# razayunus/ManhattanSLAM

Hardware: AMD Instinct MI355X
Metric: RGB-D frames/sec at 640x480 (ORB+surfel front end) (higher is better)
Workload: dtype u8/i32 (ORB)/f32+f64 (surfel)

## Files before the change

manhattanslam_amd/csrc/msl_sf.h:

```cpp
#pragma once

#include "msl_common.h"

#include <hip/hip_ext.h>

namespace msl {
namespace sf {

constexpr int SP = 8;
constexpr int NCHUNK = 10;
constexpr double MAX_ANGLE_COS = 0.1, HUBER_RANGE = 0.4, MIN_TOLERATE_DIFF = 0.1;
constexpr unsigned T_INF = 0xFFFFFFFFu;
constexpr int PROP_ROUNDS = 6;
constexpr unsigned short IDX_NONE = 0xFFFF, IDX_PLANE = 0xFFFE;
constexpr int LIST_D = 256;
constexpr int SCAN_ITEMS = 1024;
#ifndef MSL_SUB_ITEMS
#define MSL_SUB_ITEMS 128
#endif
constexpr int SUB_ITEMS = MSL_SUB_ITEMS;
constexpr int DEFER_WIN = 32;
#ifndef MSL_FUSEREC_PLANES
#define MSL_FUSEREC_PLANES 0
#endif
__host__ __device__ inline size_t fuserec_index(int nseeds, unsigned seed, int word) {
#if MSL_FUSEREC_PLANES
    return (size_t)word * (size_t)nseeds + seed;
#else
    (void)nseeds; return 3 * (size_t)seed + (size_t)word;
#endif
}

struct alignas(16) HotPk { float px, py, pz; unsigned tl; };
struct HotRec { float px, py, pz; int updateTimes, lastUpdate; };
constexpr unsigned HOT_WIDE = 0x80000000u, HOT_HOLE = 0xFFFFFFFFu;
__host__ __device__ inline bool tl_fits(int ut, int lu) { return (unsigned)ut < 2048u && ((unsigned)lu + (1u << 19)) < (1u << 20); }
__host__ __device__ inline unsigned tl_pack(int ut, int lu) { return ((unsigned)ut << 20) | ((unsigned)lu & 0xFFFFFu); }
__host__ __device__ inline int tl_ut(unsigned tl) { return (int)(tl >> 20); }
__host__ __device__ inline int tl_lu(unsigned tl) { return (int)(tl << 12) >> 12; }
struct alignas(32) ColdRec { float nx, ny, nz, size, color, weight; unsigned rgbf; unsigned _spare; };
constexpr unsigned COLD_WIDE = 1u << 24;
struct MapSoA {
    HotPk *hot;
    ColdRec *cold;
    int *rgbWide;
    int *utlWide;
    long long *wideFlag;
};
__host__ __device__ inline bool rgb_fits(int r, int g, int b) { return ((unsigned)r | (unsigned)g | (unsigned)b) < 256u; }
__host__ __device__ inline unsigned rgb_pack(int r, int g, int b) { return (unsigned)r | ((unsigned)g << 8) | ((unsigned)b << 16); }

template <typename T> using gptr = const T __attribute__((address_space(1))) *;
struct FrameDev {
    const uint8_t *gray; const float *depth; const int32_t *member;
    float pose[16], invPose[16];
    int ref, _pad;
#ifdef __HIPCC__
    __device__ __forceinline__ gptr<uint8_t> grayG() const { return (gptr<uint8_t>)gray; }
    __device__ __forceinline__ gptr<float> depthG() const { return (gptr<float>)depth; }
    __device__ __forceinline__ gptr<int32_t> memberG() const { return (gptr<int32_t>)member; }
#endif
};

struct alignas(32) AssignRec {
    float x, y, meanIntensity;
    unsigned stable;
    double invDepth;
    unsigned long long _pad;
};

struct FuseAux {
    MapSoA map;
    unsigned long long cap;
// ... 179 lines not shown
```

manhattanslam_amd/csrc/msl_sf_map.hip:

```cpp

#include "msl_sf.h"

using namespace msl;
using namespace msl::sf;

namespace {

__device__ __forceinline__ unsigned ld_agent(const unsigned *p) { return __hip_atomic_load(p, __ATOMIC_RELAXED, __HIP_MEMORY_SCOPE_AGENT); }
__device__ __forceinline__ void st_agent(unsigned *p, unsigned v) { __hip_atomic_store(p, v, __ATOMIC_RELAXED, __HIP_MEMORY_SCOPE_AGENT); }
__device__ __forceinline__ unsigned long long ld_agent64(const unsigned long long *p) { return __hip_atomic_load(p, __ATOMIC_RELAXED, __HIP_MEMORY_SCOPE_AGENT); }
__device__ __forceinline__ void st_agent64(unsigned long long *p, unsigned long long v) { __hip_atomic_store(p, v, __ATOMIC_RELAXED, __HIP_MEMORY_SCOPE_AGENT); }

__device__ __forceinline__ void set_wide_flag_ptr(long long *flag, unsigned long long bit) { atomicOr(reinterpret_cast<unsigned long long *>(flag), bit); }
__device__ __forceinline__ void set_wide_flag(const MapSoA &M, unsigned long long bit) { set_wide_flag_ptr(M.wideFlag, bit); }
__device__ __forceinline__ void tl_unpack(const MapSoA &M, long long i, unsigned tl, int &ut, int &lu) {
    ut = tl_ut(tl); lu = tl_lu(tl);
    if (tl & 0x80000000u) {
        if (tl == HOT_WIDE) { ut = M.utlWide[2 * i]; lu = M.utlWide[2 * i + 1]; }
        else { ut = 0; lu = 0; }
    }
}
__device__ __forceinline__ HotRec hot_load(const MapSoA &M, long long i) {
    const HotPk p = M.hot[i];
    HotRec h; h.px = p.px; h.py = p.py; h.pz = p.pz;
// ... 39 lines not shown
    ColdRec c; c.nx = e.nx; c.ny = e.ny; c.nz = e.nz; c.size = e.size; c.color = e.color; c.weight = e.weight; c._spare = 0;
    if (rgb_fits(e.r, e.g, e.b)) c.rgbf = rgb_pack(e.r, e.g, e.b);
    else { c.rgbf = COLD_WIDE; set_wide_flag(M, 1ull); M.rgbWide[3 * i] = e.r; M.rgbWide[3 * i + 1] = e.g; M.rgbWide[3 * i + 2] = e.b; }
    hot_store(M, i, h); cold_store(M.cold + i, c);
}
__device__ __forceinline__ void load_surfel(const MapSoA &M, long long i, const HotRec &h, msl_surfel &e) {
    const ColdRec c = cold_load(M.cold + i);
    e.px = h.px; e.py = h.py; e.pz = h.pz; e.nx = c.nx; e.ny = c.ny; e.nz = c.nz; e.size = c.size; e.color = c.color;
    if (c.rgbf & COLD_WIDE) { e.r = M.rgbWide[3 * i]; e.g = M.rgbWide[3 * i + 1]; e.b = M.rgbWide[3 * i + 2]; }
    else { e.r = (int)(c.rgbf & 255u); e.g = (int)((c.rgbf >> 8) & 255u); e.b = (int)((c.rgbf >> 16) & 255u); }
    e.weight = c.weight; e.updateTimes = h.updateTimes; e.lastUpdate = h.lastUpdate;
}
__device__ __forceinline__ void move_surfel(const MapSoA &M, long long dst, long long src) {
    const ColdRec c = cold_load(M.cold + src);
    const HotPk p = M.hot[src];
    M.hot[dst] = p; cold_store(M.cold + dst, c);
    if (p.tl == HOT_WIDE) { M.utlWide[2 * dst] = M.utlWide[2 * src]; M.utlWide[2 * dst + 1] = M.utlWide[2 * src + 1]; }
    if (c.rgbf & COLD_WIDE) { M.rgbWide[3 * dst] = M.rgbWide[3 * src]; M.rgbWide[3 * dst + 1] = M.rgbWide[3 * src + 1]; M.rgbWide[3 * dst + 2] = M.rgbWide[3 * src + 2]; }
}

__device__ __forceinline__ bool last_workgroup(unsigned *ticket, unsigned *s_flag) {
    asm volatile("s_waitcnt vmcnt(0)" ::: "memory");
    __syncthreads();
    if (threadIdx.x == 0) {
        const unsigned t = atomicAdd(ticket, 1u);
        *s_flag = (t == gridDim.x - 1) ? 1u : 0u;
        if (*s_flag) __hip_atomic_store(ticket, 0u, __ATOMIC_RELAXED, __HIP_MEMORY_SCOPE_AGENT);
    }
    __syncthreads();
    return *s_flag != 0;
}

__device__ __forceinline__ int round_half_up_pixel(float u) {
    const float c = fminf(fmaxf(u, -4.0f), 1.0e6f);
    const float f = floorf(c);
    return (int)f + ((c - f) >= 0.5f ? 1 : 0);
}
__device__ __forceinline__ unsigned lane_rank(unsigned long long m) {
    return __builtin_amdgcn_mbcnt_hi((unsigned)(m >> 32), __builtin_amdgcn_mbcnt_lo((unsigned)m, 0u));
}

typedef unsigned u32x4 __attribute__((ext_vector_type(4)));
__device__ __forceinline__ void st16(void *p, u32x4 v) { *reinterpret_cast<u32x4 *>(p) = v; }

struct FuseFrame {
    float inv[12];
    int ref;
    const FrameDev *frame;
};
struct FuseArgs {
    int W, H, nseeds, kf;
    int prevSlot;
    int rowScale;
    float fx, fy, cx, cy, fuseFar, fuseNear;
    const uint2 *tex; const float4 *fuseRec; uint8_t *fused;
    HotPk *hot; ColdRec *cold;
    long long *ctr;
    unsigned *blockSums, *blockUpd;
    unsigned *sbKeys;
    const unsigned *deal;
    unsigned *delOut;
    unsigned *delCount;
    DeferCtl *dc;
};
__host__ inline FuseArgs fuse_args(const SfDev &P, int slot, bool deferred, bool dealt = false) {
    FuseArgs A;
    A.W = P.W; A.H = P.H; A.nseeds = P.nseeds; A.kf = P.kf; A.prevSlot = P.prevSlotAbs; A.rowScale = (254 << 16) / P.H;
    A.sbKeys = P.sbKeys; A.deal = dealt ? P.deal : nullptr;
    A.fx = P.fx; A.fy = P.fy; A.cx = P.cx; A.cy = P.cy; A.fuseFar = P.fuseFar; A.fuseNear = P.fuseNear;
    A.tex = P.tex + (size_t)slot * P.pxStride; A.fuseRec = P.fuseRec + (size_t)slot * P.nseeds * 3; A.fused = P.fused + (size_t)slot * P.flagStride;
    A.hot = P.map.hot; A.cold = P.map.cold; A.ctr = P.ctr;
    A.dc = P.dc;
    A.blockSums = P.blockSums; A.blockUpd = P.blockUpd + (size_t)(deferred ? P.kf : 0) * (P.cap / SUB_ITEMS + 8200);
    A.delOut = deferred ? P.delList : P.delU;
    A.delCount = deferred ? &P.dc->delCnt[P.kf < DEFER_WIN ? P.kf : 0] : P.delUCount;
    return A;
}
__host__ inline FuseFrame fuse_frame(const FrameDev &F, const FrameDev *dev) {
    FuseFrame f;
    for (int c = 0; c < 4; c++) for (int r = 0; r < 3; r++) f.inv[3 * c + r] = F.invPose[4 * c + r];
    f.ref = F.ref; f.frame = dev;
    return f;
}
__device__ __forceinline__ void mul4r(const float *m, float v0, float v1, float v2, float v3, float out[3]) {
#pragma unroll
    for (int r = 0; r < 3; r++) out[r] = ((m[r] * v0 + m[3 + r] * v1) + m[6 + r] * v2) + m[9 + r] * v3;
}
__device__ __forceinline__ void mul3r(const float *m, float v0, float v1, float v2, float out[3]) {
#pragma unroll
    for (int r = 0; r < 3; r++) out[r] = (m[r] * v0 + m[3 + r] * v1) + m[6 + r] * v2;
}

__device__ __forceinline__ unsigned spawn_word(unsigned fw) { return ~(fw | (fw >> 1)) & 0x01010101u; }
__device__ __forceinline__ unsigned spawn_count(const FuseArgs &P, unsigned lane, unsigned &excl) {
    const DeferCtl *dc = P.dc;
    const int fs = dc->flagStride;
    const uint8_t *fusedP = dc->fused + (size_t)P.prevSlot * fs;
    const int per = fs >> 6, nch = per >> 4;
    unsigned cnt = 0;
    const uint4 *fq = reinterpret_cast<const uint4 *>(fusedP + (size_t)lane * per);
    for (int c = 0; c < nch; c += 5) {
        uint4 b[5];
#pragma unroll
        for (int q = 0; q < 5; q++) b[q] = fq[min(c + q, nch - 1)];
#pragma unroll
        for (int q = 0; q < 5; q++)
            if (c + q < nch) cnt += (unsigned)(__popc(spawn_word(b[q].x)) + __popc(spawn_word(b[q].y)) + __popc(spawn_word(b[q].z)) + __popc(spawn_word(b[q].w)));
    }
    const unsigned incl = wave_incl_scan(cnt);
    excl = incl - cnt;
    return (unsigned)__builtin_amdgcn_readlane((int)incl, 63);
}
__device__ __forceinline__ void emit_records(const FuseArgs &P, long long E0, long long c0, int nj, unsigned lane, unsigned K, unsigned excl) {
    const DeferCtl *dc = P.dc;
    const int fs = dc->flagStride;
    const uint8_t *fusedP = dc->fused + (size_t)P.prevSlot * fs;
    const int per = fs >> 6, nch = per >> 4;
    const msl_surfel *cand = dc->cand + (size_t)P.prevSlot * P.nseeds;
#pragma unroll 1
    for (int j = 0; j < nj; j++) {
        const long long i = c0 + 64 * j + lane, kS = i - E0;
        const bool on = kS >= 0 && kS < (long long)K;
        const unsigned k = on ? (unsigned)kS : 0u;
        unsigned lo = 0, hi = 63, eLo = 0;
#pragma unroll
        for (int s = 0; s < 6; s++) {
            const unsigned mid = (lo + hi + 1) >> 1;
            const unsigned e = (unsigned)__builtin_amdgcn_ds_bpermute((int)(mid * 4u), (int)excl);
            if (e <= k) { lo = mid; eLo = e; } else hi = mid - 1;
        }
        unsigned r = k - eLo;
        int seed = -1;
        const uint4 *of = reinterpret_cast<const uint4 *>(fusedP + (size_t)lo * per);
        for (int c = 0; c < nch; c++) {
            const uint4 b = of[c];
            const unsigned w[4] = {spawn_word(b.x), spawn_word(b.y), spawn_word(b.z), spawn_word(b.w)};
#pragma unroll
            for (int q = 0; q < 4; q++) {
                const unsigned pc = (unsigned)__popc(w[q]);
                if (seed < 0) {
                    if (r < pc) {
                        unsigned m = w[q];
                        for (unsigned t = 0; t < r; t++) m &= m - 1;
                        seed = (int)lo * per + 16 * c + 4 * q + (__builtin_ctz(m) >> 3);
                    } else r -= pc;
                }
            }
        }
        if (on && seed >= 0) {
            if ((unsigned long long)i < dc->aux.cap) store_surfel(dc->aux.map, i, cand[seed]);
            else { long long code = 20; asm volatile("" : "+v"(code)); P.ctr[5] = code; }
        }
    }
    asm volatile("s_waitcnt vmcnt(0)" ::: "memory");
}

template <bool DEFER, bool spawnWave>
__device__ __forceinline__ void fuse_body(const FuseArgs &P, const FuseFrame &F, int nSubHint, unsigned waveIdx, int G) {
    constexpr int KPL = SUB_ITEMS / 64;
    constexpr long long WSPAN = 64 * KPL;
    struct { HotPk *hot; ColdRec *cold; } M = {P.hot, P.cold};
    const FuseAux *aux = &P.dc->aux;
    const unsigned lane0 = threadIdx.x;
    const uint2 *tex = P.tex;
    const float4 *fuseRec = P.fuseRec;
    uint8_t *fused = P.fused;
    const int ref = F.ref;
    const float cameraF = (float)(((double)fabsf(P.fx) + (double)fabsf(P.fy)) / 2.0);
    const float halfF = 0.5f * cameraF;
    const bool pending = DEFER && P.kf > 0;
    long long E0v = 0;
    if (pending) E0v = P.dc->ext[P.kf - 1];
    long long E0 = 0;
    if (DEFER && spawnWave) E0 = ((long long)__builtin_amdgcn_readfirstlane((int)(E0v >> 32)) << 32) | (unsigned)__builtin_amdgcn_readfirstlane((int)E0v);
    if (spawnWave && !pending) return;
    if (DEFER && !pending && waveIdx == 0 && lane0 == 0) P.dc->ext[0] = P.ctr[0];
    if (DEFER && !spawnWave && waveIdx == 0 && lane0 == 0) P.dc->logBase[P.kf] = P.kf > 0 ? P.dc->logBase[P.kf - 1] + P.dc->delCnt[P.kf - 1] : 0u;
    unsigned spK = 0;
    if (DEFER && spawnWave) {
        unsigned excl;
        spK = spawn_count(P, lane0, excl);
        if (lane0 == 0) P.dc->ext[P.kf] = E0 + (long long)spK;
        if (spK == 0) return;
    }
#ifndef MSL_FUSE_CHUNK
#define MSL_FUSE_CHUNK 16
#endif
    constexpr unsigned FUSE_CHUNK = MSL_FUSE_CHUNK;
    long long sb0;
    if (!spawnWave && P.deal != nullptr) {
        const unsigned gs = (unsigned)G >> 3;
        const unsigned *dp = P.deal + ((waveIdx & 7u) * gs + (waveIdx >> 3));
        unsigned dv;
        asm volatile("s_load_dword %0, %1, 0x0\n\ts_waitcnt lgkmcnt(0)" : "=s"(dv) : "s"(dp) : "memory");
        sb0 = (long long)dv;
    } else {
        long long lin = waveIdx;
        constexpr unsigned T = 8u * FUSE_CHUNK;
        const unsigned full = ((unsigned)G / T) * T;
        if (waveIdx < full) { const unsigned grp = waveIdx / T, r = waveIdx % T; lin = (long long)grp * T + (r & 7u) * FUSE_CHUNK + (r >> 3); }
        sb0 = (long long)G - 1 - lin;
    }
    for (long long it = 0;; it++) {
        unsigned lane = lane0;
        asm volatile("" : "+v"(lane));
#define REC_LOCAL(k) (64u * (unsigned)(k) + lane)
        const long long sb = sb0 + it * G;
        long long c0, n = 0, cntIdx;
        if (DEFER && spawnWave) {
            c0 = E0 + it * WSPAN;
            n = E0 + (long long)spK;
            if (c0 >= n) return;
            unsigned excl;
            (void)spawn_count(P, lane, excl);
            emit_records(P, E0, c0, KPL, lane, spK, excl);
            cntIdx = E0 / SUB_ITEMS + 1 + it;
        } else {
            c0 = sb * WSPAN; cntIdx = sb;
            if (pending) {
                if (it > 0) {
                    E0 = ((long long)__builtin_amdgcn_readfirstlane((int)(E0v >> 32)) << 32) | (unsigned)__builtin_amdgcn_readfirstlane((int)E0v);
                    if (c0 >= E0) return;
                }
            } else if (sb >= nSubHint && c0 >= __hip_atomic_load(&P.ctr[0], __ATOMIC_RELAXED, __HIP_MEMORY_SCOPE_AGENT)) return;
        }
        HotPk hq[KPL];
#pragma unroll
        for (int k = 0; k < KPL; k++) hq[k] = M.hot[c0 + REC_LOCAL(k)];
        if (!pending) n = P.ctr[0];
        else if (!spawnWave) {
            E0 = ((long long)__builtin_amdgcn_readfirstlane((int)(E0v >> 32)) << 32) | (unsigned)__builtin_amdgcn_readfirstlane((int)E0v);
            if (c0 >= E0) return;
            n = E0;
        }
        unsigned stp = 0;
        unsigned keyAcc = 0;
        float pzv[KPL];
        unsigned offT[KPL];
        unsigned anyTl = 0;
#pragma unroll
        for (int k = 0; k < KPL; k++) anyTl |= hq[k].tl;
        const bool anyHi = __builtin_expect(__ballot(anyTl >> 31) != 0ull, 0);
#pragma unroll
        for (int k = 0; k < KPL; k++) {
            const long long i = c0 + REC_LOCAL(k);
            const float x = hq[k].px, y = hq[k].py, z = hq[k].pz;
            const unsigned tl = hq[k].tl;
            int ut = tl_ut(tl), lu = tl_lu(tl);
            bool hole = false;
            if (anyHi) {
                if (tl == HOT_WIDE) { const int *w = aux->map.utlWide; ut = w[2 * i]; lu = w[2 * i + 1]; }
                else if (tl & 0x80000000u) hole = true;
            }
            float pc[3];
            mul4r(F.inv, x, y, z, 1.0f, pc);
            const bool inRange = !(pc[2] < P.fuseNear || pc[2] > P.fuseFar);
            const bool live = i < n && !hole, stale = ref - lu > 5 && ut < 5;
            int st = 0;
            if (live) st = stale ? (ut != 0 ? 1 : 2) : (ut == 0 ? 2 : 0);
            const bool cand = live && !stale && ut != 0 && inRange;
            unsigned off = 0;
            {
                const float zq = inRange ? pc[2] : 1.0f;
                const float projectU = pc[0] * P.fx / zq + P.cx, projectV = pc[1] * P.fy / zq + P.cy;
                const int pUInt = round_half_up_pixel(projectU), pVInt = round_half_up_pixel(projectV);
                const bool inImage = !(pUInt < 1 || pUInt > P.W - 2 || pVInt < 1 || pVInt > P.H - 2);
                if (cand && inImage) { st = 3; keyAcc += (((unsigned)pVInt * (unsigned)P.rowScale) >> 16) | 0x10000u; }
                off = st == 3 ? (unsigned)(pVInt * P.W + pUInt) : 0u;
            }
            stp |= (unsigned)st << (2 * k); pzv[k] = pc[2];
            offT[k] = off;
        }
        uint2 tx[KPL];
        {
#pragma unroll
            for (int k = 0; k < KPL; k++) tx[k] = tex[offT[k]];
            if constexpr (KPL == 4) asm volatile("" ::"v"(tx[0].x), "v"(tx[1].x), "v"(tx[2].x), "v"(tx[3].x), "v"(tx[0].y), "v"(tx[1].y), "v"(tx[2].y), "v"(tx[3].y));
            else asm volatile("" ::"v"(tx[0].x), "v"(tx[KPL - 1].x), "v"(tx[0].y), "v"(tx[KPL - 1].y));
        }
        if (!(DEFER && spawnWave)) {
            const unsigned ks = (unsigned)__builtin_amdgcn_readlane((int)wave_incl_scan(keyAcc), 63);
            const unsigned kc = ks >> 16;
            const unsigned key = kc ? min((unsigned)((float)(ks & 0xFFFFu) * __builtin_amdgcn_rcpf((float)kc)), 254u) : 255u;
            if (lane == 0) P.sbKeys[cntIdx] = key;
        }
        unsigned fl = 0;
        unsigned cntDel = 0;
#pragma unroll
        for (int k = 0; k < KPL; k++) {
            const unsigned st = (stp >> (2 * k)) & 3u;
            const bool occluded = st == 3u && (double)pzv[k] < (double)__uint_as_float(tx[k].x) - 1.0;
            const bool del = st == 1u || st == 2u || occluded;
            if (DEFER) { if (del) M.hot[c0 + REC_LOCAL(k)].tl = HOT_HOLE; }
            else if (st == 1u || occluded) {
                if (__builtin_expect(hq[k].tl == HOT_WIDE, 0)) aux->map.utlWide[2 * (c0 + REC_LOCAL(k))] = 0;
                else M.hot[c0 + REC_LOCAL(k)].tl = hq[k].tl & 0xFFFFFu;
            }
            fl |= del ? (1u << k) : 0u;
            fl |= (st == 3u && !occluded) ? (16u << k) : 0u;
            cntDel += (unsigned)__popcll(__ballot(del));
        }
        auto list_base = [&](unsigned c) -> unsigned {
            unsigned base = 0, prior = 0;
            if (DEFER && P.kf > 0) prior = P.dc->logBase[P.kf - 1] + P.dc->delCnt[P.kf - 1];
            if (lane == 0) base = atomicAdd(P.delCount, c);
            return (unsigned)__builtin_amdgcn_readfirstlane((int)base) + prior;
        };
        auto hand_over = [&](bool d, unsigned long long m, unsigned base, long long i) {
            if (d) {
                const unsigned j = base + lane_rank(m);
                if (DEFER || j < (unsigned)LIST_D) P.delOut[j] = (unsigned)i;
            }
        };
        if (cntDel) {
            unsigned base = list_base(cntDel);
#pragma unroll
            for (int k = 0; k < KPL; k++) {
                const bool d = (fl >> k) & 1u;
                const unsigned long long m = __ballot(d);
                hand_over(d, m, base, c0 + REC_LOCAL(k)); base += (unsigned)__popcll(m);
            }
        }
        unsigned rcv[KPL], bk[KPL];
        unsigned total = 0;
#pragma unroll
        for (int k = 0; k < KPL; k++) {
            const bool sv = (fl >> (4 + k)) & 1u;
            const unsigned long long m = __ballot(sv);
            const unsigned c = (unsigned)__popcll(m), rs = lane_rank(m);
// ... 44 lines not shown
                        const float newWeight = f1.w;
                        const float sumWeight = oldWeight + newWeight;
                        const float fusedPx = (h.px * oldWeight + newWeight * f1.x) / sumWeight;
                        const float fusedPy = (h.py * oldWeight + newWeight * f1.y) / sumWeight;
                        const float fusedPz = (h.pz * oldWeight + newWeight * f1.z) / sumWeight;
                        float fusedNx = nc[0] * oldWeight + newWeight * f0.x;
                        float fusedNy = nc[1] * oldWeight + newWeight * f0.y;
                        float fusedNz = nc[2] * oldWeight + newWeight * f0.z;
                        const float newNormLength = sqrtf(fusedNx * fusedNx + fusedNy * fusedNy + fusedNz * fusedNz);
                        fusedNx = fusedNx / newNormLength; fusedNy = fusedNy / newNormLength; fusedNz = fusedNz / newNormLength;
                        float newNormW[3];
                        newNormW[0] = (r00 * fusedNx + r01 * fusedNy) + r02 * fusedNz;
                        newNormW[1] = (r10 * fusedNx + r11 * fusedNy) + r12 * fusedNz;
                        newNormW[2] = (r20 * fusedNx + r21 * fusedNy) + r22 * fusedNz;
                        int ut = (int)(h.tl >> 20);
                        if (__builtin_expect(h.tl == HOT_WIDE, 0)) ut = aux->map.utlWide[2 * i];
                        unsigned tlNew = tl_pack(ut + 1, ref);
                        if (__builtin_expect(!tl_fits(ut + 1, ref), 0)) {
                            int *w = aux->map.utlWide;
                            w[2 * i] = ut + 1; w[2 * i + 1] = ref;
                            asm volatile("" ::: "memory");
                            set_wide_flag_ptr(aux->map.wideFlag, 2ull);
                            tlNew = HOT_WIDE;
                        }
                        c.rgbf = __float_as_uint(f2.z);
                        c.nx = newNormW[0]; c.ny = newNormW[1]; c.nz = newNormW[2];
                        c.weight = sumWeight;
                        c.color = f2.y;
                        const float newSize = f2.x;
                        if (newSize < c.size) c.size = newSize;
                        u32x4 hv = {__float_as_uint(fusedPx), __float_as_uint(fusedPy), __float_as_uint(fusedPz), tlNew};
                        u32x4 c0v = {__float_as_uint(c.nx), __float_as_uint(c.ny), __float_as_uint(c.nz), __float_as_uint(c.size)};
                        u32x4 c1v = {__float_as_uint(c.color), __float_as_uint(c.weight), c.rgbf, 0u};
                        st16(M.hot + i, hv);
                        st16(M.cold + i, c0v);
                        st16(reinterpret_cast<u32x4 *>(M.cold + i) + 1, c1v);
                        fused[sp] = 1;
                        upd = true;
                    }
                }
            }
            nupd += (unsigned)__popcll(__ballot(upd));
            const unsigned long long mb = __ballot(delB);
            if (mb) {
                const unsigned cb = (unsigned)__popcll(mb);
                hand_over(delB, mb, list_base(cb), i);
                cntDelB += cb;
            }
        }
        if (lane == 0) {
            if (!DEFER) P.blockSums[cntIdx] = cntDel + cntDelB;
            P.blockUpd[cntIdx] = nupd;
        }
        if (!(DEFER && spawnWave) && (sb + G) * WSPAN >= n) return;
    }
#undef REC_LOCAL
}

template <bool DEFER>
__global__ __launch_bounds__(64) __attribute__((amdgpu_waves_per_eu(6, 8))) void k_fuse(FuseArgs P, FuseFrame F, int nSubHint) {
    __builtin_amdgcn_s_setprio(3);
    if (DEFER) {
        if (blockIdx.x == 0) fuse_body<DEFER, true>(P, F, nSubHint, 0u, (int)gridDim.x - 1);
        else fuse_body<DEFER, false>(P, F, nSubHint, blockIdx.x - 1u, (int)gridDim.x - 1);
    } else {
        fuse_body<false, false>(P, F, nSubHint, blockIdx.x, (int)gridDim.x);
    }
}

template <int NT>
__device__ __forceinline__ void deal_subblocks(const unsigned *keys, int G, unsigned *deal, unsigned *s_hist, unsigned *s_off, unsigned *s_wave, unsigned *s_aux) {
    static_assert(NT == 256, "one histogram bin per thread");
    const unsigned t = threadIdx.x;
    constexpr int CH = 32 * NT;
    auto load_pack = [&](int base, unsigned (&kp)[8]) {
        uint4 v[8];
#pragma unroll
        for (int q = 0; q < 8; q++) v[q] = *reinterpret_cast<const uint4 *>(keys + base + 32 * (int)t + 4 * q);
#pragma unroll
        for (int q = 0; q < 8; q++) kp[q] = min(v[q].x, 255u) | (min(v[q].y, 255u) << 8) | (min(v[q].z, 255u) << 16) | (min(v[q].w, 255u) << 24);
    };
    auto next_word = [&](unsigned (&kp)[8]) -> unsigned {
        const unsigned w = kp[0];
#pragma unroll
        for (int q = 0; q < 7; q++) kp[q] = kp[q + 1];
        kp[7] = w;
        return w;
    };
    auto count_chunk = [&](int base, unsigned (&kp)[8], bool hist) -> unsigned {
        unsigned fc = 0;
#pragma unroll 1
        for (int d = 0; d < 8; d++) {
            const unsigned w = next_word(kp);
#pragma unroll
            for (int b = 0; b < 4; b++) {
                const unsigned key = (w >> (8 * b)) & 255u;
                const bool in = base + 32 * (int)t + 4 * d + b < G;
                if (hist && in && key != 255u) atomicAdd(&s_hist[key], 1u);
                fc += in && key == 255u ? 1u : 0u;
            }
        }
        return fc;
    };
    unsigned k0[8];
    load_pack(0, k0);
    s_hist[t] = 0;
    __syncthreads();
    const unsigned fc0 = count_chunk(0, k0, true);
    for (int base = CH; base < G; base += CH) { unsigned kc[8]; load_pack(base, kc); (void)count_chunk(base, kc, true); }
    __syncthreads();
    unsigned NI, fTot0, ex, fb0;
    block_excl_scan_pair(t < 255u ? s_hist[t] : 0u, fc0, s_wave, &NI, &fTot0, ex, fb0);
    const unsigned gs = (unsigned)G >> 3;
    auto inS = [&](unsigned x) { return (x * NI + 7u) >> 3; };
    auto outS = [&](unsigned x) { return x * gs - inS(x); };
    {
        unsigned x0 = 0;
#pragma unroll
        for (unsigned y = 1; y < 8; y++) x0 += ex >= inS(y) ? 1u : 0u;
// ... 700 lines not shown
    load_surfel(M, i, h, e);
    dst[i] = e;
}
__global__ void k_set_ctr(long long *ctr, long long n, unsigned *delUCount, int wide) {
    if (threadIdx.x == 0) {
        delUCount[0] = 0;
        ctr[0] = n; ctr[1] = 0; ctr[2] = 0; ctr[3] = 0; ctr[4] = n; ctr[6] = n; ctr[7] = 0;
        if (wide >= 0) ctr[13] = wide;
    }
}

__global__ __launch_bounds__(64) void k_collect_changed(SfDev P, int ref, long long n, unsigned *count, unsigned *idxOut, msl_surfel *recOut, unsigned capOut) {
    const long long sb = blockIdx.x;
    if (!(P.blockSums[sb] | P.blockUpd[sb])) return;
    const unsigned lane = threadIdx.x;
    for (int k = 0; k < SUB_ITEMS / 64; k++) {
        const long long i = sb * SUB_ITEMS + k * 64 + lane;
        HotRec h; h.px = h.py = h.pz = 0; h.updateTimes = 1; h.lastUpdate = ref - 1;
        if (i < n) h = hot_load(P.map, i);
        const bool ch = i < n && (h.updateTimes == 0 || h.lastUpdate == ref);
        const unsigned long long m = __ballot(ch);
        if (!m) continue;
        unsigned base = 0;
        if (lane == 0) base = atomicAdd(count, (unsigned)__popcll(m));
        base = __builtin_amdgcn_readfirstlane(base);
        if (ch) {
            const unsigned j = base + lane_rank(m);
            if (j < capOut) { msl_surfel e; load_surfel(P.map, i, h, e); recOut[j] = e; idxOut[j] = (unsigned)i; }
        }
    }
}

__global__ void k_empty(int grid_dummy) { (void)grid_dummy; }

}

namespace msl {
namespace sf {

void map_launch_deal(hipStream_t st, const SfDev &P) { hipLaunchKernelGGL(k_deal, dim3(1), dim3(256), 0, st, P.sbKeys, P.dealG, P.deal); }
int map_debug_deal(const uint32_t *keys_host, int G, uint32_t *deal_host) {
    if (!keys_host || !deal_host || G < 8 || (G & 7)) return MSL_ERR_INVALID;
    const size_t pad = (size_t)G + 8192;
    DevBuf keys, deal;
    MSL_HIP_TRY(grow_all(0, {{keys, sizeof(unsigned) * pad}, {deal, sizeof(unsigned) * (G + 64)}}));
    unsigned *dk = (unsigned *)keys.p, *dd = (unsigned *)deal.p;
    MSL_HIP_TRY(hipMemset(dk, 0xFF, sizeof(unsigned) * pad)); MSL_HIP_TRY(hipMemset(dd, 0xFF, sizeof(unsigned) * G));
    MSL_HIP_TRY(hipMemcpy(dk, keys_host, sizeof(unsigned) * G, hipMemcpyHostToDevice));
    hipLaunchKernelGGL(k_deal, dim3(1), dim3(256), 0, 0, dk, G, dd);
    MSL_HIP_TRY(hipGetLastError());
    MSL_HIP_TRY(hipMemcpy(deal_host, dd, sizeof(unsigned) * G, hipMemcpyDeviceToHost));
    return MSL_OK;
}
void map_launch_fuse(KernelProfiler &prof, hipStream_t st, const SfDev &P, int slot, const FrameDev &F, int nSubGrid, int nSubHint, bool deferred, bool dealt) {
    const FuseArgs A = fuse_args(P, slot, deferred, dealt);
    const FuseFrame FF = fuse_frame(F, P.frames + slot);
    if (deferred) MSL_SF_LAUNCH(prof, SK_FUSE, st, k_fuse<true>, dim3((unsigned)nSubGrid + 1u), dim3(64), A, FF, nSubHint);
    else MSL_SF_LAUNCH(prof, SK_FUSE, st, k_fuse<false>, dim3((unsigned)nSubGrid), dim3(64), A, FF, nSubHint);
}
void map_launch_compact(KernelProfiler &prof, hipStream_t st, const SfDev &P, int slot, bool resident) {
    const CompactArgs A = compact_args(P, slot);
    const int per = (((P.nseeds + 255) / 256) + 3) & ~3;
    const bool aligned4 = (P.nseeds & 3) == 0 && ((reinterpret_cast<size_t>(A.candOk) | reinterpret_cast<size_t>(A.fused)) & 3) == 0;
    const dim3 grid(resident ? 128 : 1);
    if (per <= 32 && aligned4) MSL_SF_LAUNCH(prof, SK_COMPACT, st, k_compact<8>, grid, dim3(256), A, resident ? 0 : 1);
    else if (per <= 96 && aligned4) MSL_SF_LAUNCH(prof, SK_COMPACT, st, k_compact<24>, grid, dim3(256), A, resident ? 0 : 1);
    else MSL_SF_LAUNCH(prof, SK_COMPACT, st, k_compact<0>, grid, dim3(256), A, resident ? 0 : 1);
}
void map_launch_replay(KernelProfiler &prof, hipStream_t st, const SfDev &P, int F, unsigned blkStride) {
    const unsigned nFront = (unsigned)((P.nseeds + SUB_ITEMS - 1) / SUB_ITEMS) + 1u;
    hipLaunchKernelGGL(k_defer_tail, dim3((unsigned)F + nFront), dim3(64), 0, st, P, fuse_args(P, 0, true), F, blkStride);
    MSL_SF_LAUNCH(prof, SK_COMPACT, st, k_replay, dim3(1), dim3(64), P, F);
    hipLaunchKernelGGL(k_gather, dim3(128), dim3(256), 0, st, P);
    hipLaunchKernelGGL(k_scatter, dim3(128), dim3(256), 0, st, P);
}
void map_launch_empty_pair(KernelProfiler &prof, hipStream_t st) {
    hipEvent_t ea, eb;
    if (prof.kernel_pair(SK_NEW, &ea, &eb)) hipExtLaunchKernelGGL(k_empty, dim3(1), dim3(64), 0, st, ea, eb, 0, 0);
}
void map_launch_set_ctr(hipStream_t st, const SfDev &P, long long n, int wide) { hipLaunchKernelGGL(k_set_ctr, dim3(1), dim3(64), 0, st, P.ctr, n, P.delUCount, wide); }
void map_launch_add_ctr(hipStream_t st, const SfDev &P, long long add) { hipLaunchKernelGGL(k_add_ctr, dim3(1), dim3(64), 0, st, P.ctr, add); }
void map_launch_aos_to_soa(KernelProfiler &prof, hipStream_t st, const SfDev &P, const msl_surfel *src, long long n, bool atEnd) {
    if (atEnd) hipLaunchKernelGGL(k_aos_to_soa_at, dim3((unsigned)((n + 255) / 256)), dim3(256), 0, st, P.map, src, n, P.ctr);
    else MSL_SF_LAUNCH(prof, SK_CONVERT, st, k_aos_to_soa, dim3((unsigned)((n + 255) / 256)), dim3(256), P.map, src, n);
}
void map_launch_soa_to_aos(KernelProfiler &prof, hipStream_t st, const SfDev &P, msl_surfel *dst, long long n) {
    MSL_SF_LAUNCH(prof, SK_CONVERT, st, k_soa_to_aos, dim3((unsigned)((n + 255) / 256)), dim3(256), P.map, dst, n);
}
void map_launch_select_count(hipStream_t st, const SfDev &P, int mode, int arg) {
    hipLaunchKernelGGL(k_select_count, dim3(512), dim3(256), 0, st, P, mode, arg);
    hipLaunchKernelGGL(k_select_scan, dim3(1), dim3(1024), 0, st, P);
}
void map_launch_select_write(hipStream_t st, const SfDev &P, int mode, int arg, msl_surfel *out, int markDeleted) {
    hipLaunchKernelGGL(k_select_write, dim3(512), dim3(256), 0, st, P, mode, arg, out, markDeleted);
}
void map_launch_collect_changed(hipStream_t st, const SfDev &P, int ref, long long n, unsigned *count, unsigned *idxOut, msl_surfel *recOut, unsigned capOut) {
    const unsigned nblk = (unsigned)((n + SUB_ITEMS - 1) / SUB_ITEMS);
    hipLaunchKernelGGL(k_collect_changed, dim3(nblk), dim3(64), 0, st, P, ref, n, count, idxOut, recOut, capOut);
}
void map_launch_empty(hipStream_t st, int grid, hipEvent_t a, hipEvent_t b) { hipExtLaunchKernelGGL(k_empty, dim3((unsigned)grid), dim3(64), 0, st, a, b, 0, grid); }

}
}
```

manhattanslam_amd/csrc/msl_surfel.hip:

```cpp

#include "msl_sf.h"

#include <algorithm>
#include <cmath>
#include <cstdlib>
#include <fstream>
#include <memory>
#include <new>
#include <vector>

using namespace msl;
using namespace msl::sf;

namespace {
const char *kSfNames[MSL_SF_NKERNELS] = {"kb_seed_init", "kb_assign", "kb_prop", "kb_commit_px", "kb_update_seeds", "kb_commit_seeds",
                                         "kb_seed_plane", "k_fuse", "k_empty", "k_compact", "k_convert", "copy"};
}

struct msl_sf {
    int device = 0;
    SfDev dev{};
    int maxBatch = 1;
    hipStream_t preStream = nullptr, mapStream = nullptr; bool ownStreams = true;
    size_t blkStride = 0;
    unsigned long long kfClassic = 0, kfDeferred = 0;
    int dealG = 0;
    hipStream_t copyStream = nullptr;
    hipEvent_t evH2D[2] = {nullptr, nullptr};
    hipEvent_t evPre[2] = {nullptr, nullptr}, evMap[2] = {nullptr, nullptr}, evCopy[2] = {nullptr, nullptr};
    bool evMapValid[2] = {false, false}, evCopyValid[2] = {false, false}, evPreValid[2] = {false, false};
    unsigned long long batchNo = 0;
    int stagedSet = -1; size_t stagedGs = 0;
    int lastSlot = 0;
    struct Slots {
        DevBuf frames, seeds, seedsTmp, cand, candOk, fused, tex, fuseRec, index, amap, tmin, arec, pxInv, wl, wlCount, chunkAbort, changed;
        PinBuf hFrames;
        DevBuf gray, depth, member;
        size_t grayCap = 0, depthCap = 0, memberCap = 0;
        DevBuf depth16; size_t depth16Cap = 0;
    } slot;
    DevBuf d_ctr; PinBuf h_ctr;
    DevBuf d_tickets, d_delU, d_dc, d_projTab;
    bool propLds = false;
    bool classicNext = true;
    DevBuf d_new;
    struct MapBufs { DevBuf store, blockSums, blockUpd, delList, srcOf, rp; } map;
    size_t liveBound = 0;
    size_t liveKnown = 0;
    unsigned long long liveKnownKf = 0;
    static constexpr int NSNAP = 4;
    static constexpr int SNAPW = 16;
    PinBuf h_snap; hipEvent_t snapEv[NSNAP] = {}; unsigned long long snapKf[NSNAP] = {}; bool snapBusy[NSNAP] = {};
    bool snapLive[NSNAP] = {};
    unsigned long long kfEnq = 0; int snapNext = 0;
    long long churnNew = -1, churnDel = 0, churnKf = 0; unsigned long long churnAt = 0; double churn = 0.0;
    DevBuf d_aos;
    DevBuf d_snapStore; size_t snapN = 0; bool snapValid = false; long long snapWide = 0;
    bool mirrorValid = false; size_t mirrorN = 0;
    PinBuf h_blk;
    PinBuf h_list;
    KernelProfiler prof;
};

namespace {

constexpr size_t MAP_WORDS = 17, RP_WORDS = 24;
void set_map_ptrs(msl_sf *h, size_t c) {
    MapSoA &M = h->dev.map;
    float *store = (float *)h->map.store.p;
    M.hot = reinterpret_cast<HotPk *>(store);
    M.cold = reinterpret_cast<ColdRec *>(store + 4 * c);
    M.rgbWide = reinterpret_cast<int *>(store + 12 * c);
    M.utlWide = reinterpret_cast<int *>(store + 15 * c);
    M.wideFlag = h->dev.ctr + 13;
    SfDev &D = h->dev;
    D.cap = c;
    D.blockSums = (unsigned *)h->map.blockSums.p; D.blockUpd = (unsigned *)h->map.blockUpd.p; D.delList = (unsigned *)h->map.delList.p; D.srcOf = (unsigned *)h->map.srcOf.p;
    D.sbKeys = D.blockSums + h->blkStride; D.deal = D.blockSums + 2 * h->blkStride; D.dealG = 0;
    unsigned *r = (unsigned *)h->map.rp.p;
// ... 223 lines not shown
    }
    if (d16 && mem != MSL_MEM_HOST) {
        if (db > S.depthCap) {
            int rc = sync_all(h);
            if (rc != MSL_OK) return rc;
            S.gray = DevBuf(); S.depth = DevBuf(); S.member = DevBuf(); S.grayCap = S.depthCap = S.memberCap = 0;
            MSL_HIP_TRY(S.depth.grow(db * slots, sm));
            S.depthCap = db;
        }
        sp_launch_depth_u16(sp, depth16, d16s, d16fs, (float *)((uint8_t *)S.depth.p + (size_t)slot0 * S.depthCap), S.depthCap / 4, W, H, n, depthFactor);
    }
    const uint8_t *sd = (const uint8_t *)S.depth.p;
    if (h->evCopyValid[set]) MSL_HIP_TRY(hipEventSynchronize(h->evCopy[set]));
    FrameDev *hf = (FrameDev *)S.hFrames.p;
    for (int f = 0; f < n; f++) {
        FrameDev &F = hf[slot0 + f];
        const size_t s = slot0 + f;
        if (mem == MSL_MEM_HOST) {
            F.gray = (const uint8_t *)S.gray.p + s * S.grayCap; F.depth = (const float *)(sd + s * S.depthCap);
            F.member = (const int32_t *)((const uint8_t *)S.member.p + (mfs == 0 ? (size_t)slot0 : s) * S.memberCap);
        } else {
            F.gray = gray + f * gfs; F.member = (const int32_t *)((const uint8_t *)member + f * mfs);
            F.depth = d16 ? (const float *)(sd + s * S.depthCap) : (const float *)((const uint8_t *)depth + f * dfs);
        }
        memcpy(F.pose, poses + 16 * f, sizeof(float) * 16);
        inverse4<float>(F.pose, F.invPose);
        F.ref = refs[f]; F._pad = 0;
    }
    MSL_HIP_TRY(hipMemcpyAsync((FrameDev *)S.frames.p + slot0, hf + slot0, sizeof(FrameDev) * n, hipMemcpyHostToDevice, sp));
    MSL_HIP_TRY(hipEventRecord(h->evCopy[set], sp));
    h->evCopyValid[set] = true;

    SfDev P = D;
    P.frames = D.frames + slot0; P.seeds = D.seeds + (size_t)slot0 * D.nseeds; P.seedsTmp = D.seedsTmp + (size_t)slot0 * D.nseeds;
    P.cand = D.cand + (size_t)slot0 * D.nseeds; P.candOk = D.candOk + (size_t)slot0 * D.flagStride; P.fused = D.fused + (size_t)slot0 * D.flagStride;
    P.tex = D.tex + (size_t)slot0 * D.pxStride; P.fuseRec = D.fuseRec + (size_t)slot0 * D.nseeds * 3;
    P.index = D.index + (size_t)slot0 * D.pxStride; P.amap = D.amap + (size_t)slot0 * D.pxStride; P.tmin = D.tmin + (size_t)slot0 * D.nseeds;
    P.arec = D.arec + (size_t)slot0 * D.nseeds; P.pxInv = D.pxInv + (size_t)slot0 * D.pxStride; P.wl = D.wl + (size_t)slot0 * D.pxStride; P.wlCount = D.wlCount + slot0;
    P.chunkAbort = D.chunkAbort + slot0 * 32; P.changed = D.changed + slot0 * 8;
    sp_launch_stage(h->prof, sp, P, n, h->propLds);
    if (sp != sm) {
        MSL_HIP_TRY(hipEventRecord(h->evPre[set], sp));
        h->evPreValid[set] = true;
        MSL_HIP_TRY(hipStreamWaitEvent(sm, h->evPre[set], 0));
    }
    const size_t boundLive = compact ? h->liveBound : D.cap;
    const size_t known = std::min(h->liveKnown, boundLive);
    const size_t subWant = (std::min(known + 2 * (size_t)D.nseeds, boundLive) + SUB_ITEMS - 1) / SUB_ITEMS;
    const int nSubGrid = (int)std::max<size_t>(8, std::min((subWant + 63) & ~(size_t)63, (size_t)D.cap / SUB_ITEMS));
    const int nSubHint = (int)(known / SUB_ITEMS);
    static const int DEAL_EVERY = getenv("MSL_SF_DEAL_EVERY") ? std::max(1, atoi(getenv("MSL_SF_DEAL_EVERY"))) : 4;
    static const char *dealEnv = getenv("MSL_SF_DEAL");
    constexpr int DEAL_MAX_GRID = (4 << 20) / SUB_ITEMS;
    const bool dealOn = !(dealEnv && !strcmp(dealEnv, "0")) && (nSubGrid & 7) == 0 && (size_t)nSubGrid <= h->blkStride && nSubGrid <= DEAL_MAX_GRID;
    static const char *deferEnv = getenv("MSL_SF_DEFER");
    static const bool deferOff = deferEnv && !strcmp(deferEnv, "0"), deferForce = deferEnv && !strcmp(deferEnv, "1");
    constexpr double CHURN_MAX = 96.0;
    const bool churny = !deferForce && (h->churn > CHURN_MAX || sp != sm);
    auto classic = [&](int f) {
        P.kf = 0;
        map_launch_fuse(h->prof, sm, P, f, hf[slot0 + f], nSubGrid, nSubHint, false, dealOn && h->dealG == nSubGrid);
        P.dealG = dealOn && compact && (f % DEAL_EVERY == 0 || h->dealG != nSubGrid) ? nSubGrid : 0;
        map_launch_compact(h->prof, sm, P, f, compact);
        if (P.dealG) h->dealG = nSubGrid;
        h->kfClassic++;
    };
    int f = 0;
    const int fProbe = n / 2;
    if (!compact || deferOff || churny || n < 2) {
        for (; f < n; f++) { classic(f); if (f == fProbe) map_launch_empty_pair(h->prof, sm); }
    } else {
        if (h->classicNext) { classic(0); f = 1; if (fProbe == 0) map_launch_empty_pair(h->prof, sm); }
        while (f < n) {
            const int w = std::min(DEFER_WIN, n - f);
            for (int q = 0; q < w; q++) {
                P.kf = q; P.prevSlotAbs = slot0 + f + q - 1;
                map_launch_fuse(h->prof, sm, P, f + q, hf[slot0 + f + q], nSubGrid, nSubHint, true, dealOn && h->dealG == nSubGrid);
                if (f + q == fProbe) map_launch_empty_pair(h->prof, sm);
            }
            P.kf = w; P.prevSlotAbs = slot0 + f + w - 1;
            map_launch_replay(h->prof, sm, P, w, (unsigned)h->blkStride);
            h->kfDeferred += (unsigned long long)w;
            if (dealOn) { P.dealG = nSubGrid; map_launch_deal(sm, P); h->dealG = nSubGrid; }
            f += w;
        }
    }
    if (compact) h->classicNext = false;
    if (sp != sm) { MSL_HIP_TRY(hipEventRecord(h->evMap[set], sm)); h->evMapValid[set] = true; }
    if (compact && h->h_snap.p) {
        const int i = h->snapNext;
        if (!h->snapBusy[i]) {
            MSL_HIP_TRY(hipMemcpyAsync((long long *)h->h_snap.p + (size_t)i * msl_sf::SNAPW, D.ctr, sizeof(long long) * msl_sf::SNAPW, hipMemcpyDeviceToHost, sm));
            MSL_HIP_TRY(hipEventRecord(h->snapEv[i], sm));
            h->snapKf[i] = h->kfEnq; h->snapBusy[i] = true; h->snapLive[i] = true; h->snapNext = (i + 1) % msl_sf::NSNAP;
        }
    }
    MSL_HIP_TRY(hipGetLastError());
    h->lastSlot = slot0 + n - 1;
    h->batchNo++;
    return MSL_OK;
}

}

extern "C" {

msl_sf *msl_sf_create(int width, int height, float fx, float fy, float cx, float cy, float fuseFar, float fuseNear, int device) noexcept {
    try {
    if (width < 16 || height < 16 || fx == 0 || fy == 0 || (width / SP) * (height / SP) >= IDX_PLANE || (long long)width * height >= (1ll << 31)) {
        set_error("msl_sf_create: width/height must be >= 16 with fewer than 65534 superpixels, fx and fy non-zero");
        return nullptr;
    }
    if (bind_device(device) != MSL_OK) return nullptr;
    std::unique_ptr<msl_sf, void (*)(msl_sf *)> guard(new msl_sf, [](msl_sf *p) { msl_sf_destroy(p); });
    msl_sf *h = guard.get();
    h->device = device;
    SfDev &D = h->dev;
    D.W = width; D.H = height; D.spW = width / SP; D.spH = height / SP; D.nseeds = D.spW * D.spH; D.npx = width * height;
    D.pxStride = (D.npx + 63) & ~63;
    D.flagStride = 64 * ((((D.nseeds + 63) / 64) + 15) & ~15);
    D.fx = fx; D.fy = fy; D.cx = cx; D.cy = cy; D.fuseFar = fuseFar; D.fuseNear = fuseNear;
    bool ok = true;
    {
        int lo = 0, hi = 0;
        ok = ok && hipDeviceGetStreamPriorityRange(&lo, &hi) == hipSuccess;
        ok = ok && hipStreamCreateWithPriority(&h->preStream, hipStreamNonBlocking, lo) == hipSuccess;
        ok = ok && hipStreamCreateWithPriority(&h->mapStream, hipStreamNonBlocking, hi) == hipSuccess;
        ok = ok && hipStreamCreateWithFlags(&h->copyStream, hipStreamNonBlocking) == hipSuccess;
    }
    for (int i = 0; i < 2 && ok; i++)
        ok = hipEventCreateWithFlags(&h->evPre[i], hipEventDisableTiming) == hipSuccess && hipEventCreateWithFlags(&h->evMap[i], hipEventDisableTiming) == hipSuccess &&
             hipEventCreateWithFlags(&h->evCopy[i], hipEventDisableTiming) == hipSuccess &&
             hipEventCreateWithFlags(&h->evH2D[i], hipEventDisableTiming) == hipSuccess;
    const hipStream_t sm = h->mapStream;
    ok = ok && h->d_ctr.grow(sizeof(long long) * 32, sm) == hipSuccess;
    ok = ok && hipMemset(h->d_ctr.p, 0, sizeof(long long) * 32) == hipSuccess;
    ok = ok && h->h_ctr.grow(sizeof(long long) * 16, sm) == hipSuccess;
    ok = ok && h->h_snap.grow(sizeof(long long) * msl_sf::NSNAP * msl_sf::SNAPW, sm) == hipSuccess;
    for (int i = 0; i < msl_sf::NSNAP && ok; i++) ok = hipEventCreateWithFlags(&h->snapEv[i], hipEventDisableTiming) == hipSuccess;
    ok = ok && h->d_new.grow(sizeof(msl_surfel) * D.nseeds, sm) == hipSuccess;
    ok = ok && h->d_tickets.grow(sizeof(unsigned) * 8, sm) == hipSuccess && hipMemset(h->d_tickets.p, 0, sizeof(unsigned) * 8) == hipSuccess;
    ok = ok && h->d_delU.grow(sizeof(unsigned) * LIST_D, sm) == hipSuccess;
    ok = ok && h->d_dc.grow(sizeof(DeferCtl), sm) == hipSuccess && hipMemset(h->d_dc.p, 0, sizeof(DeferCtl)) == hipSuccess;
    {
        std::vector<float> tab((size_t)width + 1 + height + 1);
        for (int u = 0; u <= width; u++) tab[u] = ((float)u - cx) / fx;
        for (int v = 0; v <= height; v++) tab[(size_t)width + 1 + v] = ((float)v - cy) / fy;
        ok = ok && h->d_projTab.grow(sizeof(float) * tab.size(), sm) == hipSuccess;
        ok = ok && hipMemcpy(h->d_projTab.p, tab.data(), sizeof(float) * tab.size(), hipMemcpyHostToDevice) == hipSuccess;
        D.colX = (const float *)h->d_projTab.p; D.rowY = D.colX + width + 1;
    }
    if (ok) h->propLds = sp_init_attributes(D.nseeds);
    if (!ok) { set_error("msl_sf_create: HIP allocation failed"); return nullptr; }
    memset(h->h_ctr.p, 0, sizeof(long long) * 16);
    D.ctr = (long long *)h->d_ctr.p; D.newSurfels = (msl_surfel *)h->d_new.p; D.tickets = (unsigned *)h->d_tickets.p; D.delU = (unsigned *)h->d_delU.p;
    D.delUCount = D.tickets + 4; D.dc = (DeferCtl *)h->d_dc.p; D.kf = 0; D.prevSlotAbs = 0;
    h->prof.nk = MSL_SF_NKERNELS;
    if (alloc_slots(h, 1) != MSL_OK || map_realloc(h, 1 << 16, 0) != MSL_OK) return nullptr;
    return guard.release();
    } MSL_ABI_CATCH_PTR
}

void msl_sf_destroy(msl_sf *h) noexcept {
    try {
    if (!h) return;
    (void)hipSetDevice(h->device);
    if (h->copyStream) (void)hipStreamSynchronize(h->copyStream);
    if (h->preStream) (void)hipStreamSynchronize(h->preStream);
    if (h->mapStream) (void)hipStreamSynchronize(h->mapStream);
// ... 519 lines not shown
```

Before: 25730.

## Let fuse waves walk several consecutive sub-blocks and gate dealing on 8-XCD devices

Adds a template parameter S so each fuse wave processes S consecutive sub-blocks of a run, with a prefetch touch of the next sub-block's hot records. The launch grid shrinks by S, and an environment variable selects S. The default is 1, so the existing per-wave mapping is kept. Separately, the XCD-aware dealing of sub-blocks is now enabled only when the device reports 8 XCCs. The multi-block walk is meant to cut wave launch overhead and improve locality, at the cost of more complex termination logic.

```diff
diff --git a/manhattanslam_amd/csrc/msl_sf.h b/manhattanslam_amd/csrc/msl_sf.h
--- a/manhattanslam_amd/csrc/msl_sf.h
+++ b/manhattanslam_amd/csrc/msl_sf.h
@@ -19,6 +19,7 @@
 #define MSL_SUB_ITEMS 128
 #endif
 constexpr int SUB_ITEMS = MSL_SUB_ITEMS;
+constexpr int FUSE_WALK_DEFAULT = 1;
 constexpr int DEFER_WIN = 32;
 #ifndef MSL_FUSEREC_PLANES
 #define MSL_FUSEREC_PLANES 0
diff --git a/manhattanslam_amd/csrc/msl_sf_map.hip b/manhattanslam_amd/csrc/msl_sf_map.hip
--- a/manhattanslam_amd/csrc/msl_sf_map.hip
+++ b/manhattanslam_amd/csrc/msl_sf_map.hip
@@ -115,6 +115,7 @@
     int W, H, nseeds, kf;
     int prevSlot;
     int rowScale;
+    int nSub;
     float fx, fy, cx, cy, fuseFar, fuseNear;
     const uint2 *tex; const float4 *fuseRec; uint8_t *fused;
     HotPk *hot; ColdRec *cold;
@@ -128,7 +129,7 @@
 };
 __host__ inline FuseArgs fuse_args(const SfDev &P, int slot, bool deferred, bool dealt = false) {
     FuseArgs A;
-    A.W = P.W; A.H = P.H; A.nseeds = P.nseeds; A.kf = P.kf; A.prevSlot = P.prevSlotAbs; A.rowScale = (254 << 16) / P.H;
+    A.W = P.W; A.H = P.H; A.nseeds = P.nseeds; A.kf = P.kf; A.prevSlot = P.prevSlotAbs; A.rowScale = (254 << 16) / P.H; A.nSub = 0;
     A.sbKeys = P.sbKeys; A.deal = dealt ? P.deal : nullptr;
     A.fx = P.fx; A.fy = P.fy; A.cx = P.cx; A.cy = P.cy; A.fuseFar = P.fuseFar; A.fuseNear = P.fuseNear;
     A.tex = P.tex + (size_t)slot * P.pxStride; A.fuseRec = P.fuseRec + (size_t)slot * P.nseeds * 3; A.fused = P.fused + (size_t)slot * P.flagStride;
@@ -218,7 +219,7 @@
     asm volatile("s_waitcnt vmcnt(0)" ::: "memory");
 }
 
-template <bool DEFER, bool spawnWave>
+template <bool DEFER, bool spawnWave, int S>
 __device__ __forceinline__ void fuse_body(const FuseArgs &P, const FuseFrame &F, int nSubHint, unsigned waveIdx, int G) {
     constexpr int KPL = SUB_ITEMS / 64;
     constexpr long long WSPAN = 64 * KPL;
@@ -250,35 +251,61 @@
 #define MSL_FUSE_CHUNK 16
 #endif
     constexpr unsigned FUSE_CHUNK = MSL_FUSE_CHUNK;
-    long long sb0;
-    if (!spawnWave && P.deal != nullptr) {
-        const unsigned gs = (unsigned)G >> 3;
-        const unsigned *dp = P.deal + ((waveIdx & 7u) * gs + (waveIdx >> 3));
-        unsigned dv;
-        asm volatile("s_load_dword %0, %1, 0x0\n\ts_waitcnt lgkmcnt(0)" : "=s"(dv) : "s"(dp) : "memory");
-        sb0 = (long long)dv;
-    } else {
-        long long lin = waveIdx;
-        constexpr unsigned T = 8u * FUSE_CHUNK;
-        const unsigned full = ((unsigned)G / T) * T;
-        if (waveIdx < full) { const unsigned grp = waveIdx / T, r = waveIdx % T; lin = (long long)grp * T + (r & 7u) * FUSE_CHUNK + (r >> 3); }
-        sb0 = (long long)G - 1 - lin;
-    }
-    for (long long it = 0;; it++) {
+    static_assert(FUSE_CHUNK % S == 0 && (S & (S - 1)) == 0, "a wave walks S consecutive sub-blocks of one run");
+    const bool dealt = !spawnWave && P.deal != nullptr;
+    long long sb0 = 0;
+    unsigned lin0 = 0;
+    if constexpr (S == 1) {
+        if (dealt) {
+            const unsigned gs = (unsigned)G >> 3;
+            const unsigned *dp = P.deal + ((waveIdx & 7u) * gs + (waveIdx >> 3));
+            unsigned dv;
+            asm volatile("s_load_dword %0, %1, 0x0\n\ts_waitcnt lgkmcnt(0)" : "=s"(dv) : "s"(dp) : "memory");
+            sb0 = (long long)dv;
+        } else {
+            long long lin = waveIdx;
+            constexpr unsigned T = 8u * FUSE_CHUNK;
+            const unsigned full = ((unsigned)G / T) * T;
+            if (waveIdx < full) { const unsigned grp = waveIdx / T, r = waveIdx % T; lin = (long long)grp * T + (r & 7u) * FUSE_CHUNK + (r >> 3); }
+            sb0 = (long long)G - 1 - lin;
+        }
+    } else if (!dealt) {
+        constexpr unsigned T = 8u * FUSE_CHUNK, TW = T / S;
+        const unsigned full = ((unsigned)G / T) * T, fullW = full / S;
+        lin0 = full + (waveIdx - fullW) * S;
+        if (waveIdx < fullW) { const unsigned grp = waveIdx / TW, r = waveIdx % TW; lin0 = grp * T + (r & 7u) * FUSE_CHUNK + (r >> 3) * S; }
+    }
+    typedef const __attribute__((address_space(4))) unsigned *ConstU;
+    auto step_sb = [&](unsigned it) -> int {
+        const unsigned t = it % S, m = it / S;
+        unsigned b;
+        if (dealt) {
+            const unsigned R = (unsigned)G >> 3, Q = (R + S - 1) / S, e = (waveIdx >> 3) + t * Q;
+            if (e >= R) return -1;
+            b = ((ConstU)P.deal)[(waveIdx & 7u) * R + e];
+        } else {
+            if (lin0 + t >= (unsigned)G) return -1;
+            b = (unsigned)G - 1u - (lin0 + t);
+        }
+        return (int)(b + m * (unsigned)G);
+    };
+    int sbNext = S > 1 ? step_sb(0) : 0;
+    bool more = false;
+    for (unsigned it = 0;; it++) {
         unsigned lane = lane0;
         asm volatile("" : "+v"(lane));
 #define REC_LOCAL(k) (64u * (unsigned)(k) + lane)
-        const long long sb = sb0 + it * G;
-        long long c0, n = 0, cntIdx;
+        long long sb = 0, c0, n = 0, cntIdx;
         if (DEFER && spawnWave) {
-            c0 = E0 + it * WSPAN;
+            c0 = E0 + (long long)it * WSPAN;
             n = E0 + (long long)spK;
             if (c0 >= n) return;
             unsigned excl;
             (void)spawn_count(P, lane, excl);
             emit_records(P, E0, c0, KPL, lane, spK, excl);
             cntIdx = E0 / SUB_ITEMS + 1 + it;
-        } else {
+        } else if constexpr (S == 1) {
+            sb = sb0 + (long long)it * G;
             c0 = sb * WSPAN; cntIdx = sb;
             if (pending) {
                 if (it > 0) {
@@ -286,6 +313,22 @@
                     if (c0 >= E0) return;
                 }
             } else if (sb >= nSubHint && c0 >= __hip_atomic_load(&P.ctr[0], __ATOMIC_RELAXED, __HIP_MEMORY_SCOPE_AGENT)) return;
+        } else {
+            if (it > 0 && it % S == 0) {
+                if (!more) return;
+                more = false;
+            }
+            sb = sbNext; c0 = sb * WSPAN; cntIdx = sb;
+            bool skip = sbNext < 0;
+            if (!skip) {
+                if (pending) {
+                    if (it > 0) {
+                        E0 = ((long long)__builtin_amdgcn_readfirstlane((int)(E0v >> 32)) << 32) | (unsigned)__builtin_amdgcn_readfirstlane((int)E0v);
+                        skip = c0 >= E0;
+                    }
+                } else skip = sb >= nSubHint && c0 >= __hip_atomic_load(&P.ctr[0], __ATOMIC_RELAXED, __HIP_MEMORY_SCOPE_AGENT);
+            }
+            if (skip) { sbNext = step_sb(it + 1); continue; }
         }
         HotPk hq[KPL];
 #pragma unroll
@@ -293,9 +336,14 @@
         if (!pending) n = P.ctr[0];
         else if (!spawnWave) {
             E0 = ((long long)__builtin_amdgcn_readfirstlane((int)(E0v >> 32)) << 32) | (unsigned)__builtin_amdgcn_readfirstlane((int)E0v);
-            if (c0 >= E0) return;
+            if (c0 >= E0) {
+                if (S == 1) return;
+                sbNext = step_sb(it + 1);
+                continue;
+            }
             n = E0;
         }
+        if (S > 1 && !spawnWave) more = more || (sb + G) * WSPAN < n;
         unsigned stp = 0;
         unsigned keyAcc = 0;
         float pzv[KPL];
@@ -335,9 +383,15 @@
             offT[k] = off;
         }
         uint2 tx[KPL];
+        unsigned touch = 0;
         {
 #pragma unroll
             for (int k = 0; k < KPL; k++) tx[k] = tex[offT[k]];
+            if (S > 1 && !spawnWave) {
+                sbNext = step_sb(it + 1);
+                const long long cT = sbNext >= 0 && sbNext < G ? (long long)sbNext * WSPAN : c0;
+                touch = reinterpret_cast<const unsigned *>(M.hot + cT)[(lane & 15u) * 32u];
+            }
             if constexpr (KPL == 4) asm volatile("" ::"v"(tx[0].x), "v"(tx[1].x), "v"(tx[2].x), "v"(tx[3].x), "v"(tx[0].y), "v"(tx[1].y), "v"(tx[2].y), "v"(tx[3].y));
             else asm volatile("" ::"v"(tx[0].x), "v"(tx[KPL - 1].x), "v"(tx[0].y), "v"(tx[KPL - 1].y));
         }
@@ -488,19 +542,20 @@
             if (!DEFER) P.blockSums[cntIdx] = cntDel + cntDelB;
             P.blockUpd[cntIdx] = nupd;
         }
-        if (!(DEFER && spawnWave) && (sb + G) * WSPAN >= n) return;
+        if (S > 1) asm volatile("" ::"v"(touch));
+        if (S == 1 && !(DEFER && spawnWave) && (sb + G) * WSPAN >= n) return;
     }
 #undef REC_LOCAL
 }
 
-template <bool DEFER>
+template <bool DEFER, int S>
 __global__ __launch_bounds__(64) __attribute__((amdgpu_waves_per_eu(6, 8))) void k_fuse(FuseArgs P, FuseFrame F, int nSubHint) {
     __builtin_amdgcn_s_setprio(3);
     if (DEFER) {
-        if (blockIdx.x == 0) fuse_body<DEFER, true>(P, F, nSubHint, 0u, (int)gridDim.x - 1);
-        else fuse_body<DEFER, false>(P, F, nSubHint, blockIdx.x - 1u, (int)gridDim.x - 1);
+        if (blockIdx.x == 0) fuse_body<DEFER, true, 1>(P, F, nSubHint, 0u, P.nSub);
+        else fuse_body<DEFER, false, S>(P, F, nSubHint, blockIdx.x - 1u, P.nSub);
     } else {
-        fuse_body<false, false>(P, F, nSubHint, blockIdx.x, (int)gridDim.x);
+        fuse_body<false, false, S>(P, F, nSubHint, blockIdx.x, P.nSub);
     }
 }
 
@@ -1307,11 +1362,29 @@
     MSL_HIP_TRY(hipMemcpy(deal_host, dd, sizeof(unsigned) * G, hipMemcpyDeviceToHost));
     return MSL_OK;
 }
+int map_fuse_walk() {
+    static const int walk = [] {
+        const char *e = getenv("MSL_SF_FUSE_WALK");
+        const int v = e ? atoi(e) : FUSE_WALK_DEFAULT;
+        return v == 1 || v == 2 || v == 4 ? v : FUSE_WALK_DEFAULT;
+    }();
+    return walk;
+}
+template <int S>
+static void launch_fuse(KernelProfiler &prof, hipStream_t st, const FuseArgs &A, const FuseFrame &FF, int nSubGrid, int nSubHint, bool deferred) {
+    const unsigned waves = (((unsigned)nSubGrid + S - 1) / S + 7u) & ~7u;
+    if (deferred) MSL_SF_LAUNCH(prof, SK_FUSE, st, (k_fuse<true, S>), dim3(waves + 1u), dim3(64), A, FF, nSubHint);
+    else MSL_SF_LAUNCH(prof, SK_FUSE, st, (k_fuse<false, S>), dim3(waves), dim3(64), A, FF, nSubHint);
+}
 void map_launch_fuse(KernelProfiler &prof, hipStream_t st, const SfDev &P, int slot, const FrameDev &F, int nSubGrid, int nSubHint, bool deferred, bool dealt) {
-    const FuseArgs A = fuse_args(P, slot, deferred, dealt);
+    FuseArgs A = fuse_args(P, slot, deferred, dealt);
+    A.nSub = nSubGrid;
     const FuseFrame FF = fuse_frame(F, P.frames + slot);
-    if (deferred) MSL_SF_LAUNCH(prof, SK_FUSE, st, k_fuse<true>, dim3((unsigned)nSubGrid + 1u), dim3(64), A, FF, nSubHint);
-    else MSL_SF_LAUNCH(prof, SK_FUSE, st, k_fuse<false>, dim3((unsigned)nSubGrid), dim3(64), A, FF, nSubHint);
+    switch (map_fuse_walk()) {
+        case 1: launch_fuse<1>(prof, st, A, FF, nSubGrid, nSubHint, deferred); break;
+        case 2: launch_fuse<2>(prof, st, A, FF, nSubGrid, nSubHint, deferred); break;
+        default: launch_fuse<4>(prof, st, A, FF, nSubGrid, nSubHint, deferred); break;
+    }
 }
 void map_launch_compact(KernelProfiler &prof, hipStream_t st, const SfDev &P, int slot, bool resident) {
     const CompactArgs A = compact_args(P, slot);
diff --git a/manhattanslam_amd/csrc/msl_surfel.hip b/manhattanslam_amd/csrc/msl_surfel.hip
--- a/manhattanslam_amd/csrc/msl_surfel.hip
+++ b/manhattanslam_amd/csrc/msl_surfel.hip
@@ -25,6 +25,7 @@
     size_t blkStride = 0;
     unsigned long long kfClassic = 0, kfDeferred = 0;
     int dealG = 0;
+    bool xcd8 = false;
     hipStream_t copyStream = nullptr;
     hipEvent_t evH2D[2] = {nullptr, nullptr};
     hipEvent_t evPre[2] = {nullptr, nullptr}, evMap[2] = {nullptr, nullptr}, evCopy[2] = {nullptr, nullptr};
@@ -354,7 +355,7 @@
     static const int DEAL_EVERY = getenv("MSL_SF_DEAL_EVERY") ? std::max(1, atoi(getenv("MSL_SF_DEAL_EVERY"))) : 4;
     static const char *dealEnv = getenv("MSL_SF_DEAL");
     constexpr int DEAL_MAX_GRID = (4 << 20) / SUB_ITEMS;
-    const bool dealOn = !(dealEnv && !strcmp(dealEnv, "0")) && (nSubGrid & 7) == 0 && (size_t)nSubGrid <= h->blkStride && nSubGrid <= DEAL_MAX_GRID;
+    const bool dealOn = h->xcd8 && !(dealEnv && !strcmp(dealEnv, "0")) && (nSubGrid & 7) == 0 && (size_t)nSubGrid <= h->blkStride && nSubGrid <= DEAL_MAX_GRID;
     static const char *deferEnv = getenv("MSL_SF_DEFER");
     static const bool deferOff = deferEnv && !strcmp(deferEnv, "0"), deferForce = deferEnv && !strcmp(deferEnv, "1");
     constexpr double CHURN_MAX = 96.0;
@@ -417,6 +418,10 @@
     std::unique_ptr<msl_sf, void (*)(msl_sf *)> guard(new msl_sf, [](msl_sf *p) { msl_sf_destroy(p); });
     msl_sf *h = guard.get();
     h->device = device;
+    {
+        int nx = 0;
+        h->xcd8 = hipDeviceGetAttribute(&nx, hipDeviceAttributeNumberOfXccs, device) == hipSuccess && nx == 8;
+    }
     SfDev &D = h->dev;
     D.W = width; D.H = height; D.spW = width / SP; D.spH = height / SP; D.nseeds = D.spW * D.spH; D.npx = width * height;
     D.pxStride = (D.npx + 63) & ~63;
```

Result: no change. 25770 (median of 6 runs) (+0.2%).
